# microsoft/VidTok

Hardware: NVIDIA H100
Metric: frames/sec encode+decode, kl_causal_488 17x256x256 (higher is better)
Workload: dtype bf16

## Files before the change

vidtok_b200/csrc/conv_tc.cu:

```cuda
#include <cuda.h>

#include <cstdio>
#include <cstdlib>
#include <cstring>
#include <mutex>
#include <string>
#include <type_traits>

#include "common.cuh"
#include "kernels.h"
#include "tc_host.h"
#include "tc_ptx.cuh"

namespace vt {

namespace {

thread_local std::string g_tc_err;

struct TcParams {
  int B, To, Ho, Wo, Co, Ti;
  int BW, BH, BT;
  int tilesW, tilesH, tilesT;
  int num_n_tiles, BN;
  long long num_tiles;
  int kt, kh, kw, Ci, num_kc;
  int st, pt, ph, pw, to_off;
  int sp;
  int t_mode, cacheT;
  int stages;
  const float* bias;
  int res_mode;
  const bf16* res;
  long long rsB, rsT, rsH, rsW;
  int resT, res_t_mode, res_pool_off;
  const bf16* res_cache;
  float ra, rb;
  void* out;
  long long osB, osT, osH, osW, osC;
  int out_f32;
  int Co_real;
  int w_batched;
  int ln_mode, ln_silu;
  const float* ln_gamma;
  const float* ln_beta;
  void* out2;
  int res_mma;
  int halo, hP, a_stages;
  uint32_t halo_bytes;
  int split, a_lo, b_lo, o_lo;
  float acc_scale;
  int kparts;
  int reg_mode, reg_zc, reg_sample;
  const float* reg_noise;
  float* reg_z;
  int* reg_idx;
  double* reg_kl;
  FsqConst reg_fsq;
  uint32_t misc_off;
};

struct TcMaps {
  CUtensorMap a[4];
  CUtensorMap c;
  CUtensorMap b;
  CUtensorMap r;
  CUtensorMap e;
};

constexpr int kConsumerWarps = 8;
constexpr int kProducerWarp = kConsumerWarps;
constexpr int kThreads = (kConsumerWarps + 4) * 32;
constexpr int kABytes = 128 * 128;
constexpr uint32_t kBarTurn = 3, kBarBias = 5;

__host__ __device__ constexpr bool ping_pong(int BN, bool split) { return !split && (BN == 64 || BN == 128); }

using namespace tcx;

struct TileCoord {
  int b, t0, h0, w0, n0;
};
__device__ __forceinline__ TileCoord decode_tile(const TcParams& p, long long tile) {
  TileCoord c;
  const int nt = (int)(tile % p.num_n_tiles);
  long long m = tile / p.num_n_tiles;
  const int tw = (int)(m % p.tilesW); m /= p.tilesW;
  const int th = (int)(m % p.tilesH); m /= p.tilesH;
  const int tt = (int)(m % p.tilesT);
  c.b = (int)(m / p.tilesT);
  c.t0 = tt * p.BT; c.h0 = th * p.BH; c.w0 = tw * p.BW; c.n0 = nt * p.BN;
  return c;
}
__device__ __forceinline__ bool tap_time(const TcParams& p, const TileCoord& tc, int a, int& tv, bool& from_cache) {
  tv = (tc.t0 + p.to_off) * p.st + a - p.pt;
  from_cache = false;
  if (tv + p.BT <= 0) {
    if (p.t_mode == 0) return false;
    if (p.t_mode == 1) { tv = 0; return true; }
    from_cache = true;
    tv = p.cacheT + tv;
    return true;
  }
  return true;
}
__device__ __forceinline__ int tile_taps(const TcParams& p, const TileCoord& tc) {
  int n = 0;
  for (int a = 0; a < p.kt; ++a) {
    int tv;
    bool from_cache;
    if (tap_time(p, tc, a, tv, from_cache)) ++n;
  }
  return n;
}

__device__ __forceinline__ float quad_sum(float v) {
  v += __shfl_xor_sync(0xffffffffu, v, 1);
  v += __shfl_xor_sync(0xffffffffu, v, 2);
  return v;
}

template <int BN, bool kSplit>
__global__ void __launch_bounds__(kThreads, 1)
conv_tc_kernel(const __grid_constant__ TcMaps maps, const TcParams p) {
  extern __shared__ uint8_t smem_raw[];
  const uint32_t smem_base = (smem_u32(smem_raw) + 1023u) & ~1023u;
  uint8_t* smem_gen = smem_raw + (smem_base - smem_u32(smem_raw));
  const int warp = threadIdx.x >> 5, lane = threadIdx.x & 31;
  const uint32_t a_bytes = kABytes;
  constexpr uint32_t b_bytes = (uint32_t)BN * 128u;
  constexpr uint32_t kPl = kSplit ? 2u : 1u;
  const uint32_t stage_bytes = kPl * (p.halo ? b_bytes : a_bytes + b_bytes);
  const uint32_t win_bytes = kPl * p.halo_bytes;
  const uint32_t ring_base = smem_base + (p.halo ? (uint32_t)p.a_stages * win_bytes : 0u);
  const uint32_t bar_base = ring_base + p.stages * stage_bytes;
  auto full_bar = [&](int s) { return bar_base + 8u * s; };
  auto empty_bar = [&](int s) { return bar_base + 8u * (p.stages + s); };
  auto fullA_bar = [&](int s) { return bar_base + 8u * (2 * p.stages + s); };
  auto emptyA_bar = [&](int s) { return bar_base + 8u * (2 * p.stages + p.a_stages + s); };
  constexpr bool kPingPong = ping_pong(BN, kSplit);
  float* sbias = reinterpret_cast<float*>(smem_gen + p.misc_off);
  float* rowbuf = sbias + 2 * 768;

  if (threadIdx.x == 0) {
    constexpr uint32_t readers = kPingPong ? kConsumerWarps / 2 : kConsumerWarps;
    for (int s = 0; s < p.stages; ++s) {
      mbar_init(full_bar(s), 1);
      mbar_init(empty_bar(s), readers);
    }
    for (int s = 0; s < p.a_stages; ++s) {
      mbar_init(fullA_bar(s), 1);
      mbar_init(emptyA_bar(s), readers);
    }
    asm volatile("fence.mbarrier_init.release.cluster;" ::: "memory");
  }
  __syncthreads();

  const int nsp = p.kh * p.kw;
  const int num_kc = p.num_kc, nstages = p.stages;
  const bool halo = p.halo != 0;
  const int res_steps = p.res_mma ? BN / 64 : 0;

  if (warp >= kProducerWarp) {
    asm volatile("setmaxnreg.dec.sync.aligned.u32 40;" ::: "memory");
    if (warp != kProducerWarp) return;
    const bool el = elect_one();
    if (el) {
      prefetch_tmap(&maps.a[0]);
      prefetch_tmap(&maps.b);
      if (p.sp == 2) { prefetch_tmap(&maps.a[1]); prefetch_tmap(&maps.a[2]); prefetch_tmap(&maps.a[3]); }
      if (p.t_mode == 2) prefetch_tmap(&maps.c);
      if (p.res_mma) { prefetch_tmap(&maps.r); prefetch_tmap(&maps.e); }
    }
    int stage = 0, sA = 0;
    uint32_t phase = 0, phA = 0;
    auto acquire = [&](uint32_t bytes) {
      mbar_wait(empty_bar(stage), phase ^ 1u);
      if (el) mbar_expect_tx(full_bar(stage), bytes);
    };
    auto advance = [&]() { if (++stage == nstages) { stage = 0; phase ^= 1u; } };
    auto load_b_planes = [&](uint32_t dst, const CUtensorMap* m, int kcol, int n, int wb_) {
      tma_load_3d(dst, m, full_bar(stage), kcol, n, wb_);
      if constexpr (kSplit) tma_load_3d(dst + b_bytes, m, full_bar(stage), p.b_lo + kcol, n, wb_);
    };
    auto load_window = [&](const CUtensorMap* m, int c0, int lo_off, int cw, int ch, int ct, int cb) {
      mbar_wait(emptyA_bar(sA), phA ^ 1u);
      if (el) {
        mbar_expect_tx(fullA_bar(sA), win_bytes);
        tma_load_5d(smem_base + (uint32_t)sA * win_bytes, m, fullA_bar(sA), c0, cw, ch, ct, cb);
        if constexpr (kSplit) tma_load_5d(smem_base + (uint32_t)sA * win_bytes + p.halo_bytes, m, fullA_bar(sA), lo_off + c0, cw, ch, ct, cb);
      }
      if (++sA == p.a_stages) { sA = 0; phA ^= 1u; }
    };
    for (long long tile = blockIdx.x; tile < p.num_tiles; tile += gridDim.x) {
      const TileCoord tc = decode_tile(p, tile);
      const int wb = p.w_batched ? tc.b : 0;
      for (int a = 0; a < p.kt; ++a) {
        int tv;
        bool from_cache;
        if (!tap_time(p, tc, a, tv, from_cache)) continue;
        if (halo) {
          const CUtensorMap* mapA = from_cache ? &maps.c : &maps.a[0];
          for (int kc = 0; kc < num_kc; ++kc) {
            load_window(mapA, kc * 64, p.a_lo, tc.w0 - p.pw, tc.h0 - p.ph, tv, tc.b);
            int kcol = a * nsp * p.Ci + kc * 64;
            for (int sp = 0; sp < nsp; ++sp, kcol += p.Ci) {
              acquire(stage_bytes);
              if (el) load_b_planes(ring_base + stage * stage_bytes, &maps.b, kcol, tc.n0, wb);
              advance();
            }
          }
        } else {
          int kcol = a * nsp * p.Ci;
          for (int bb = 0; bb < p.kh; ++bb) {
            for (int c = 0; c < p.kw; ++c, kcol += p.Ci) {
              const int dh = bb - p.ph, dw2 = c - p.pw;
              int ch, cw;
              const CUtensorMap* mapA;
              if (p.sp == 2) {
                mapA = &maps.a[(dh & 1) * 2 + (dw2 & 1)];
                ch = tc.h0 + (dh >> 1);
                cw = tc.w0 + (dw2 >> 1);
              } else {
                mapA = &maps.a[0];
                ch = tc.h0 + dh;
                cw = tc.w0 + dw2;
              }
              if (from_cache) mapA = &maps.c;
              for (int kc = 0; kc < num_kc; ++kc) {
                acquire(stage_bytes);
                if (el) {
                  const uint32_t sa = smem_base + stage * stage_bytes;
                  tma_load_5d(sa, mapA, full_bar(stage), kc * 64, cw, ch, tv, tc.b);
                  if constexpr (kSplit) tma_load_5d(sa + a_bytes, mapA, full_bar(stage), p.a_lo + kc * 64, cw, ch, tv, tc.b);
                  load_b_planes(sa + kPl * a_bytes, &maps.b, kcol + kc * 64, tc.n0, wb);
                }
                advance();
              }
            }
          }
        }
      }
      for (int g = 0; g < res_steps; ++g) {
        if (halo) {
          load_window(&maps.r, tc.n0 + g * 64, p.o_lo, tc.w0 - p.pw, tc.h0 - p.ph, tc.t0, tc.b);
          acquire(b_bytes);
          if (el) tma_load_3d(ring_base + stage * stage_bytes, &maps.e, full_bar(stage), g * 64, 0, 0);
        } else {
          acquire(kPl * a_bytes + b_bytes);
          if (el) {
            const uint32_t sa = smem_base + stage * stage_bytes;
            tma_load_5d(sa, &maps.r, full_bar(stage), tc.n0 + g * 64, tc.w0, tc.h0, tc.t0, tc.b);
            if constexpr (kSplit) tma_load_5d(sa + a_bytes, &maps.r, full_bar(stage), p.o_lo + tc.n0 + g * 64, tc.w0, tc.h0, tc.t0, tc.b);
            tma_load_3d(sa + kPl * a_bytes, &maps.e, full_bar(stage), g * 64, 0, 0);
          }
        }
        advance();
      }
    }
    return;
  }

  asm volatile("setmaxnreg.inc.sync.aligned.u32 232;" ::: "memory");
  constexpr int R = BN / 2;
  constexpr int kHalves = kPingPong ? 2 : 1;
  constexpr bool kSum = kSplit && BN <= 128;
  const int g = warp >> 2, wq = warp & 3;
  const bool leader = lane == 0;
  const uint32_t hi_b = desc_hi(1024u);
  const uint32_t hi_a = halo ? desc_hi((uint32_t)p.hP * 128u) : hi_b;
  const uint32_t a_half = halo ? 8u * (uint32_t)p.hP * 128u : 64u * 128u;
  const uint32_t a_row_off = kPingPong ? 0u : (uint32_t)g * a_half;
  const uint32_t a_pl = halo ? p.halo_bytes : a_bytes;
  const uint32_t b_addr0 = halo ? ring_base : smem_base + kPl * a_bytes;
  float acc[kHalves][R];
  float sum[kSum ? R : 1];
  int stage = 0, sA = 0, sR = 0;
  uint32_t phase = 0, phA = 0;
  int pend_stage = -1;
  bool pend_win = false;
  auto release = [&]() {
    if (leader) {
      if (pend_stage >= 0) mbar_arrive(empty_bar(pend_stage));
      if (pend_win) mbar_arrive(emptyA_bar(sR));
    }
    if (pend_win && ++sR == p.a_stages) sR = 0;
    pend_stage = -1;
    pend_win = false;
  };
  auto kstep = [&](bool a_from_stage, uint32_t a_addr, uint32_t scale, bool res, bool last_of_window) {
    mbar_wait(full_bar(stage), phase);
    if (a_from_stage) a_addr = smem_base + stage * stage_bytes + a_row_off;
    const uint32_t b_addr = b_addr0 + stage * stage_bytes;
    const uint32_t al = desc_lo(a_addr), bl = desc_lo(b_addr);
    wgmma_fence();
#pragma unroll
    for (uint32_t j = 0; j < 4u; ++j) {
      const uint64_t ah = desc(al + 2u * j, hi_a), bh = desc(bl + 2u * j, hi_b);
      wgmma_k16<BN, kSplit>(acc[0], ah, bh, j == 0 ? scale : 1u);
      if constexpr (kPingPong) wgmma_k16<BN, kSplit>(acc[1], desc(al + (a_half >> 4) + 2u * j, hi_a), bh, j == 0 ? scale : 1u);
      if constexpr (kSplit) {
        wgmma_k16<BN, kSplit>(acc[0], desc(al + (a_pl >> 4) + 2u * j, hi_a), bh, 1u);
        if (!res) wgmma_k16<BN, kSplit>(acc[0], ah, desc(bl + (b_bytes >> 4) + 2u * j, hi_b), 1u);
      }
    }
    wgmma_commit();
    wgmma_wait<1>();
    release();
    pend_stage = stage;
    pend_win = last_of_window;
    if (++stage == nstages) { stage = 0; phase ^= 1u; }
  };

  const int rbase = (kPingPong ? 0 : 64 * g) + 16 * wq + (lane >> 2);
  const int cq = 2 * (lane & 3);
  const bool res_direct = (p.res_mode == 1 && !p.res_mma);
  const bool store_a = (p.ln_mode != 1);
  const float inv_n = 1.0f / (float)BN;
  int last_n0 = -1;
  uint32_t cbuf = 1;

  int owner = 0;
  for (long long tile = blockIdx.x; tile < p.num_tiles; tile += gridDim.x, owner ^= 1) {
    const TileCoord tc = decode_tile(p, tile);
    if constexpr (kPingPong) {
      if (owner != g) {
        const int taps = tile_taps(p, tc);
        stage += taps * nsp * num_kc + res_steps;
        if ((stage / nstages) & 1) phase ^= 1u;
        stage %= nstages;
        if (halo) {
          const int nw = taps * num_kc + res_steps;
          sA += nw;
          if ((sA / p.a_stages) & 1) phA ^= 1u;
          sA %= p.a_stages;
          sR = (sR + nw) % p.a_stages;
        }
        continue;
      }
      if (tile != blockIdx.x) named_bar_sync(kBarTurn + g, kConsumerWarps * 32);
    }
    uint32_t G = 0xFFFFFFFFu;
    if constexpr (kSum) {
      if (p.kparts > 1) {
        const uint32_t nk = (uint32_t)(tile_taps(p, tc) * nsp * num_kc + res_steps);
        G = (nk + (uint32_t)p.kparts - 1u) / (uint32_t)p.kparts;
      }
#pragma unroll
      for (int i = 0; i < R; ++i) sum[i] = 0.f;
    }
    uint32_t ks = 0, accum = 0;
    auto step = [&](bool a_from_stage, uint32_t a_addr, bool res, bool last_of_window) {
      if constexpr (kSum) {
        if (ks > 0 && ks % G == 0) {
          wgmma_wait<0>();
          acc_fence(acc[0]);
          release();
#pragma unroll
          for (int i = 0; i < R; ++i) sum[i] += acc[0][i];
          accum = 0;
        }
      }
      kstep(a_from_stage, a_addr, accum, res, last_of_window);
      accum = 1;
      ++ks;
    };
    for (int a = 0; a < p.kt; ++a) {
      int tv;
      bool from_cache;
      if (!tap_time(p, tc, a, tv, from_cache)) continue;
      if (halo) {
        for (int kc = 0; kc < num_kc; ++kc) {
          mbar_wait(fullA_bar(sA), phA);
          const uint32_t win = smem_base + (uint32_t)sA * win_bytes + a_row_off;
          for (int bb = 0; bb < p.kh; ++bb)
            for (int c = 0; c < p.kw; ++c)
              step(false, win + (uint32_t)(bb * p.hP + c) * 128u, false, bb == p.kh - 1 && c == p.kw - 1);
          if (++sA == p.a_stages) { sA = 0; phA ^= 1u; }
        }
      } else {
        for (int s = nsp * num_kc; s > 0; --s) step(true, 0u, false, false);
      }
    }
    for (int gr = 0; gr < res_steps; ++gr) {
      if (halo) {
        mbar_wait(fullA_bar(sA), phA);
        step(false, smem_base + (uint32_t)sA * win_bytes + a_row_off + (uint32_t)(p.ph * p.hP + p.pw) * 128u, true, true);
        if (++sA == p.a_stages) { sA = 0; phA ^= 1u; }
      } else {
        step(true, 0u, true, false);
      }
    }
    if constexpr (kPingPong) {
      if (tile + gridDim.x < p.num_tiles) named_bar_arrive(kBarTurn + (g ^ 1), kConsumerWarps * 32);
    }
    wgmma_wait<0>();
#pragma unroll
    for (int hf = 0; hf < kHalves; ++hf) acc_fence(acc[hf]);
    release();
    if constexpr (kSum) {
#pragma unroll
      for (int i = 0; i < R; ++i) acc[0][i] += sum[i];
    }

    if (tc.n0 != last_n0) {
      last_n0 = tc.n0;
      cbuf ^= 1u;
      constexpr int nthr = kPingPong ? 128 : kConsumerWarps * 32;
      float* b_ = sbias + ((kPingPong ? 2 * g : 0) + cbuf) * 768;
      for (int i = threadIdx.x % nthr; i < BN; i += nthr) {
        b_[i] = (p.bias && tc.n0 + i < p.Co_real) ? p.bias[tc.n0 + i] : 0.f;
        if (p.ln_mode) { const float sc = (p.ln_silu && !kSplit) ? 0.5f : 1.0f; b_[256 + i] = sc * p.ln_gamma[tc.n0 + i]; b_[512 + i] = sc * p.ln_beta[tc.n0 + i]; }
      }
      named_bar_sync(kPingPong ? kBarBias + g : 1u, nthr);
    }
    const float* bias_s = sbias + ((kPingPong ? 2 * g : 0) + cbuf) * 768;
    const float* gamma_s = bias_s + 256;
    const float* beta_s = bias_s + 512;

#pragma unroll
    for (int hf = 0; hf < kHalves; ++hf) {
      float (&acc_h)[R] = acc[hf];
      int row0 = rbase + 64 * hf;
      asm volatile("" : "+r"(row0));
      bool valid[2];
      long long ooff[2];
      auto row_geom = [&](int row, int& t, int& h, int& w) {
        const int dw = halo ? (row & 7) : row % p.BW;
        const int dh = halo ? (row >> 3) : (row / p.BW) % p.BH;
        const int dt = halo ? 0 : row / (p.BW * p.BH);
        t = tc.t0 + dt; h = tc.h0 + dh; w = tc.w0 + dw;
        return (t < p.To) && (h < p.Ho) && (w < p.Wo);
      };
#pragma unroll
      for (int r = 0; r < 2; ++r) {
        int t, h, w;
        valid[r] = row_geom(row0 + 8 * r, t, h, w);
        ooff[r] = (long long)tc.b * p.osB + (long long)t * p.osT + (long long)h * p.osH + (long long)w * p.osW;
      }
      auto res_pair = [&](const bf16* rp, int c, float& x0, float& x1) {
        const uint32_t hw = *reinterpret_cast<const uint32_t*>(rp + c);
        if constexpr (kSplit) {
          const uint32_t lw = *reinterpret_cast<const uint32_t*>(rp + p.o_lo + c);
          x0 = f16_lo(hw) + f16_lo(lw);
          x1 = f16_hi(hw) + f16_hi(lw);
        } else {
          x0 = bf16_lo(hw);
// ... 268 lines not shown
  }
  if (reg && reg->mode) {
    const int need = reg->mode == 1 ? 2 * reg->zc : reg->zc;
    const bool zc_ok = reg->mode == 1 ? (reg->zc == 4 || reg->zc == 8 || reg->zc == 16) : reg->zc <= VT_MAX_FSQ;
    if (tout == DT_F32 && Co_pad == 32 && need <= p.Co && zc_ok && p.osW == 1) t.reg = *reg;
    else g_tc_err = "regularizer epilogue needs an fp32 [B,C,T,H,W] head with Cout <= 32 holding all latent channels";
  }
  auto plan = [&](bool allow_halo, int bn_cap) -> int {
    t.halo = 0; t.hP = 0; t.a_stages = 0; t.halo_bytes = 0;
    t.BN = choose_bn(Co_pad);
    if (bn_cap && t.BN > bn_cap) t.BN = bn_cap;
    if (!choose_tile(p, 128, t.BW, t.BH, t.BT)) { g_tc_err = "no tile shape"; return -1; }
    const bool geom = p.sh == 1 && p.sw == 1 && p.kh * p.kw > 1 && p.kh <= 3 && p.kw <= 3 && p.Ho == p.Hi && p.Wo == p.Wi &&
                      w_batches <= 1 && p.Wo % 8 == 0 && p.Ho % 16 == 0;
    if (allow_halo && geom) {
      t.halo = 1;
      t.BW = 8; t.BH = 16; t.BT = 1;
      t.hP = 16;
      t.halo_bytes = (uint32_t)((16 + p.kh - 1) * t.hP * 128);
      t.a_stages = 2;
    }
    const size_t stage_bytes = (size_t)cw * ((t.halo ? 0 : (size_t)kABytes) + (size_t)t.BN * 128);
    const size_t budget = 225 * 1024;
    const size_t a_ring = (size_t)t.a_stages * t.halo_bytes * cw;
    const size_t misc = (ping_pong(t.BN, split) ? 4 : 2) * 768 * 4 + (t.reg.mode ? 128 * 33 * 4 : 0);
    const size_t fixed = 1024  + misc + 16;
    if (budget < fixed + a_ring + 2 * (stage_bytes + 16)) return 1;
    int stages = (int)((budget - fixed - a_ring) / (stage_bytes + 16));
    if (stages > 8) stages = 8;
    static const int cap = [] { const char* e = getenv("VT_TC_STAGES"); return e ? atoi(e) : 0; }();
    if (cap >= 2 && stages > cap) stages = cap;
    t.stages = stages;
    const size_t bars = 8 * (2 * (size_t)stages + 2 * (size_t)t.a_stages);
    t.misc_off = (uint32_t)((a_ring + stages * stage_bytes + bars + 15) & ~(size_t)15);
    t.smem = 1024 + t.misc_off + misc;
    t.kparts = (split && t.BN <= 128 && nk >= 16) ? (nk >= 64 ? 8 : 4) : 1;
    return 0;
  };
  const bool need_row = t.ln.mode != 0;
  const int bn_pref = (split && !need_row && w_batches <= 1) ? (nk >= 128 ? 64 : (nk >= 16 ? 128 : 0)) : 0;
  int rc = plan(true, bn_pref);
  if (rc == 1) rc = plan(false, bn_pref);
  if (rc == 1 && !need_row) rc = plan(false, 128);
  if (rc == 1) return no("not enough shared memory for 2 stages");
  if (rc != 0) return false;
  bool ident_ok = true;
  if (split) {
    const float ws = p.acc_scale != 0.f ? 1.0f / p.acc_scale : 1.0f;
    t.ident_s = ilogbf(ws);
    ident_ok = t.ident_s >= 0 && t.ident_s <= 15 && ldexpf(1.0f, t.ident_s) == ws;
  }
  t.res_mma = (ident_ok && p.res_mode == 1 && p.ra == 1.0f && p.rb == 1.0f && t.BN % 64 == 0 && p.Co % 64 == 0 && p.rsW % 8 == 0 &&
               p.rsH % 8 == 0 && p.rsT % 8 == 0 && p.rsB % 8 == 0 && (((uintptr_t)p.res) & 15) == 0) ? 1 : 0;
  *out = t;
  return true;
}

cudaError_t launch_conv_tc(const TcPlan& pl, const bf16* x, const bf16* w_nk, void* out, cudaStream_t s, long long w_batch_stride) {
  if (!tmap_encoder()) { g_tc_err = "cuTensorMapEncodeTiled unavailable"; return cudaErrorNotSupported; }
  const ConvP& p = pl.p;
  const TcRegFusion& reg = pl.reg;
  const bool split = p.split != 0;
  const int cw = split ? 2 : 1;
  if (reg.mode ? (!reg.z || (reg.mode == 1 && (!reg.kl_acc || (reg.sample && !reg.noise)))) : !out) { g_tc_err = "null output"; return cudaErrorInvalidValue; }
  if (p.t_mode == 2 && (!p.cache || p.cacheT <= 0)) { g_tc_err = "cache mode without cache"; return cudaErrorInvalidValue; }
  int dev = 0;
  const cudaError_t dev_err = current_device(dev);
  if (dev_err != cudaSuccess) { g_tc_err = "no current device, or its index is out of range"; return dev_err; }
  const int Co_pad = (p.Co + 31) / 32 * 32, Kpad = p.kt * p.kh * p.kw * p.Ci;
  TcParams t;
  memset(&t, 0, sizeof(t));
  t.BW = pl.BW; t.BH = pl.BH; t.BT = pl.BT; t.BN = pl.BN;
  t.halo = pl.halo; t.hP = pl.hP; t.a_stages = pl.a_stages; t.halo_bytes = pl.halo_bytes;
  t.stages = pl.stages; t.misc_off = pl.misc_off; t.kparts = pl.kparts; t.res_mma = pl.res_mma;
  t.tilesW = (p.Wo + t.BW - 1) / t.BW; t.tilesH = (p.Ho + t.BH - 1) / t.BH; t.tilesT = (p.To + t.BT - 1) / t.BT;
  t.num_n_tiles = Co_pad / t.BN;
  t.num_tiles = (long long)p.B * t.tilesT * t.tilesH * t.tilesW * t.num_n_tiles;
  t.split = split ? 1 : 0; t.a_lo = p.Ci; t.b_lo = Kpad; t.o_lo = p.Co;
  t.acc_scale = (split && p.acc_scale != 0.f) ? p.acc_scale : 1.0f;
  t.B = p.B; t.To = p.To; t.Ho = p.Ho; t.Wo = p.Wo; t.Co = p.Co; t.Ti = p.Ti;
  t.kt = p.kt; t.kh = p.kh; t.kw = p.kw; t.Ci = p.Ci; t.num_kc = p.Ci / 64;
  t.st = p.st; t.pt = p.pt; t.ph = p.ph; t.pw = p.pw; t.to_off = p.to_off; t.sp = p.sh;
  t.t_mode = p.t_mode; t.cacheT = p.cacheT;
  t.bias = p.bias; t.res_mode = p.res_mode; t.res = (const bf16*)p.res;
  t.rsB = p.rsB; t.rsT = p.rsT; t.rsH = p.rsH; t.rsW = p.rsW; t.resT = p.resT; t.res_t_mode = p.res_t_mode; t.res_pool_off = p.res_pool_off;
  t.res_cache = (const bf16*)p.res_cache; t.ra = p.ra; t.rb = p.rb;
  t.out = out; t.osB = p.osB; t.osT = p.osT; t.osH = p.osH; t.osW = p.osW; t.osC = p.osC;
  t.out_f32 = (pl.tout == DT_F32) ? 1 : 0;
  t.Co_real = p.Co;
  t.ln_mode = pl.ln.mode; t.ln_silu = pl.ln.silu ? 1 : 0; t.ln_gamma = pl.ln.gamma; t.ln_beta = pl.ln.beta; t.out2 = pl.ln.out2;
  if (reg.mode) {
    t.reg_mode = reg.mode; t.reg_zc = reg.zc; t.reg_sample = reg.sample; t.reg_noise = reg.noise; t.reg_z = reg.z;
    t.reg_idx = reg.indices; t.reg_kl = reg.kl_acc;
    if (reg.mode == 2) t.reg_fsq = make_fsq_const(reg.zc, reg.fsq_levels);
  }
  t.w_batched = pl.w_batches > 1 ? 1 : 0;

  TcMaps maps;
  auto encode_act = [&](CUtensorMap* m, const bf16* base, int Wn, int Hn, long long sw_, long long sh_, int Tn, long long st_, long long bs) -> bool {
    cuuint64_t dims[5] = {(cuuint64_t)(cw * p.Ci), (cuuint64_t)Wn, (cuuint64_t)Hn, (cuuint64_t)Tn, (cuuint64_t)p.B};
    cuuint64_t strides[4] = {(cuuint64_t)sw_ * 2, (cuuint64_t)sh_ * 2, (cuuint64_t)st_ * 2, (cuuint64_t)bs * 2};
    cuuint32_t box[5] = {64, (cuuint32_t)t.BW, (cuuint32_t)t.BH, (cuuint32_t)t.BT, 1};
    if (t.halo) { box[1] = (cuuint32_t)t.hP; box[2] = (cuuint32_t)(16 + p.kh - 1); }
    return encode_tmap_16b(m, 5, base, dims, strides, box, "activation", g_tc_err);
  };
  if (p.sh == 1) {
    if (!encode_act(&maps.a[0], x, p.Wi, p.Hi, p.isW, p.isH, p.Ti, p.isT, p.isB)) return cudaErrorInvalidValue;
    maps.a[1] = maps.a[2] = maps.a[3] = maps.a[0];
  } else {
    for (int hp = 0; hp < 2; ++hp)
      for (int wp = 0; wp < 2; ++wp)
        if (!encode_act(&maps.a[hp * 2 + wp], x + (long long)hp * p.isH + (long long)wp * p.isW, (p.Wi - wp + 1) / 2,
                        (p.Hi - hp + 1) / 2, 2 * p.isW, 2 * p.isH, p.Ti, p.isT, p.isB))
          return cudaErrorInvalidValue;
  }
  if (p.t_mode == 2) {
    if (!encode_act(&maps.c, (const bf16*)p.cache, p.Wi, p.Hi, p.isW, p.isH, p.cacheT, p.isT, (long long)p.cacheT * p.Hi * p.Wi * p.Ci * cw)) return cudaErrorInvalidValue;
  } else {
    maps.c = maps.a[0];
  }
  {
    const int nb = pl.w_batches > 1 ? pl.w_batches : 1;
    cuuint64_t dims[3] = {(cuuint64_t)(cw * Kpad), (cuuint64_t)Co_pad, (cuuint64_t)nb};
    cuuint64_t strides[2] = {(cuuint64_t)(cw * Kpad) * 2, (cuuint64_t)(nb > 1 ? w_batch_stride : (long long)cw * Kpad * Co_pad) * 2};
    cuuint32_t box[3] = {64, (cuuint32_t)t.BN, 1};
    if (!encode_tmap_16b(&maps.b, 3, w_nk, dims, strides, box, "weights", g_tc_err)) return cudaErrorInvalidValue;
  }
  auto encode_out = [&](CUtensorMap* m, const void* base, int Tn, long long sW, long long sH, long long sT, long long sB, int bw, int bh, int bt) -> bool {
    cuuint64_t dims[5] = {(cuuint64_t)(cw * p.Co), (cuuint64_t)p.Wo, (cuuint64_t)p.Ho, (cuuint64_t)Tn, (cuuint64_t)p.B};
    cuuint64_t strides[4] = {(cuuint64_t)sW * 2, (cuuint64_t)sH * 2, (cuuint64_t)sT * 2, (cuuint64_t)sB * 2};
    cuuint32_t box[5] = {64, (cuuint32_t)bw, (cuuint32_t)bh, (cuuint32_t)bt, 1};
    return encode_tmap_16b(m, 5, base, dims, strides, box, "output/residual", g_tc_err);
  };
  maps.r = maps.a[0]; maps.e = maps.b;
  if (t.res_mma) {
    static bf16* ident_dev[2][kMaxDevices] = {{nullptr}};
    static std::mutex ident_mu;
    const int ik = split ? 1 : 0;
    {
      std::lock_guard<std::mutex> lock(ident_mu);
      if (!ident_dev[ik][dev]) {
        const int nmat = split ? 16 : 1;
        bf16* e = nullptr;
        cudaError_t err = cudaMalloc(&e, (size_t)nmat * 256 * 256 * sizeof(bf16));
        if (err != cudaSuccess) { g_tc_err = "cudaMalloc(identity)"; return err; }
        for (int i = 0; i < nmat; ++i) fill_identity_kernel<<<256, 256, 0, s>>>(e + (size_t)i * 256 * 256, ik, ldexpf(1.0f, i));
        if ((err = cudaStreamSynchronize(s)) != cudaSuccess) { cudaFree(e); g_tc_err = "identity fill"; return err; }
        ident_dev[ik][dev] = e;
      }
    }
    const bf16* ident = ident_dev[ik][dev] + (size_t)pl.ident_s * 256 * 256;
    if (!encode_out(&maps.r, p.res, p.resT, p.rsW, p.rsH, p.rsT, p.rsB, t.halo ? t.hP : t.BW, t.halo ? 16 + p.kh - 1 : t.BH, t.BT)) return cudaErrorInvalidValue;
    cuuint64_t dims[3] = {256, 256, 1};
    cuuint64_t strides[2] = {512, 256 * 512};
    cuuint32_t box[3] = {64, (cuuint32_t)t.BN, 1};
    if (!encode_tmap_16b(&maps.e, 3, ident, dims, strides, box, "identity", g_tc_err)) return cudaErrorInvalidValue;
  }
  {
    static SmemLimitOnce smem_limit;
    cudaError_t e = smem_limit.ensure(dev, 227 * 1024, conv_tc_kernel<32, false>, conv_tc_kernel<64, false>, conv_tc_kernel<128, false>,
                                      conv_tc_kernel<256, false>, conv_tc_kernel<32, true>, conv_tc_kernel<64, true>,
                                      conv_tc_kernel<128, true>, conv_tc_kernel<256, true>);
    if (e != cudaSuccess) { g_tc_err = "cudaFuncSetAttribute(smem)"; return e; }
  }
  const int num_sms = device_sms(dev);
  const unsigned grid = (unsigned)(t.num_tiles < num_sms ? t.num_tiles : num_sms);
  const double Mrows = (double)p.B * p.To * p.Ho * p.Wo;
  char det[160] = "";
  if (prof_enabled()) snprintf(det, sizeof(det), "k%d%d%d s%d%d %d->%d @%dx%dx%d tile%dx%dx%d bn%d%s ln%d r%d%s p%d t%d st%d", p.kt, p.kh, p.kw, p.st, p.sh, p.Ci, p.Co, p.To, p.Ho, p.Wo, t.BT, t.BH, t.BW, t.BN, t.halo ? " halo" : "", t.ln_mode, p.res_mode, t.res_mma ? "m" : "", split ? t.kparts : 1, p.t_mode, t.stages);
  ProfScope _ps(split ? "conv_tc3" : "conv_tc", 2.0 * Mrows * p.kt * p.kh * p.kw * p.Ci * p.Co,
                2.0 * cw * ((double)p.B * p.Ti * p.Hi * p.Wi * p.Ci) + Mrows * p.Co * (pl.tout == DT_F32 ? 4.0 : 2.0 * cw), s, det);
  auto launch = [&](auto kern) { kern<<<grid, kThreads, pl.smem, s>>>(maps, t); };
  switch (t.BN * 2 + (split ? 1 : 0)) {
    case 64: launch(conv_tc_kernel<32, false>); break;
    case 65: launch(conv_tc_kernel<32, true>); break;
    case 128: launch(conv_tc_kernel<64, false>); break;
    case 129: launch(conv_tc_kernel<64, true>); break;
    case 256: launch(conv_tc_kernel<128, false>); break;
    case 257: launch(conv_tc_kernel<128, true>); break;
    case 512: launch(conv_tc_kernel<256, false>); break;
    default: launch(conv_tc_kernel<256, true>); break;
  }
  count_launch();
  return cudaGetLastError();
}

}
```

vidtok_b200/csrc/kernels.h:

```cpp
#pragma once
#include <cuda_runtime.h>
#include <stdint.h>

#include "common.cuh"

namespace vt {

enum DType { DT_F32 = 0, DT_BF16 = 1, DT_SPLIT = 2 };
inline size_t dtype_size(DType t) { return t == DT_BF16 ? 2 : 4; }

void prof_start();
void prof_set_detail(bool on);
int prof_stop(char* buf, int cap);

cudaError_t launch_conv_simt(const ConvP& p, DType tin, DType tout, DType tres, const void* x, const float* w_kn,
                             void* out, cudaStream_t s);
cudaError_t launch_gemm_simt(DType ta, DType tb, DType tc, const void* A, const void* B, void* C, int M, int N, int K,
                             long long lda, long long sbn, long long sbk, long long ldc, int batch, long long bsA,
                             long long bsB, long long bsC, float scale, cudaStream_t s);

cudaError_t launch_layernorm(DType t, const void* x, const float* gamma, const float* beta, void* y, long long rows,
                             int C, bool silu, bool exact, cudaStream_t s);
cudaError_t launch_groupnorm(DType t, const void* x, const float* gamma, const float* beta, void* y, long long frames,
                             long long pos_per_frame, int C, bool per_position, bool silu, bool exact, float* stats,
// ... 26 lines not shown
                                  float wscale = 0.f);
cudaError_t launch_absmax(const float* w, long long n, float* out, cudaStream_t s);
inline float split_weight_scale(float maxabs, float headroom = 1.0f) {
  if (!(maxabs > 0.f)) return 1.0f;
  float sc = 1.0f;
  while (sc * maxabs * headroom < 2048.0f && sc < 1.0e30f) sc *= 2.0f;
  while (sc * maxabs * headroom >= 4096.0f && sc > 1.0e-30f) sc *= 0.5f;
  return sc;
}
constexpr float kModelWeightHeadroom = 4.0f;
cudaError_t launch_pack_w_collapsed(const float* w, bf16* out, int Co, int Co_pad, int Ci, int kt, int kh, int kw,
                                    const int* mt, const int* mh, const int* mw, int kt2, int kh2, int kw2, cudaStream_t s,
                                    float wscale = 0.f);
cudaError_t launch_time_interp2x(DType t, const void* x, void* y, int B, int T, long long hw, int C, cudaStream_t s);
cudaError_t launch_upsample_nearest(DType t, const void* x, void* y, int B, int T, int H, int W, int C, int ut, int uh,
                                    int uw, cudaStream_t s);
cudaError_t launch_cache_update(DType t, const void* x, const void* old_cache, void* new_cache, int B, int Tc, int P,
                                int off, bool first, long long frame_elems, long long x_bs, cudaStream_t s);
cudaError_t launch_ncdhw_to_cl(DType t, const float* x, void* y, int B, int C, int T, int H, int W, int t_rep,
                               cudaStream_t s);
cudaError_t launch_copy_frames(DType t, const void* src, void* dst, int B, long long src_bs, long long dst_bs,
                               long long n_per_batch, cudaStream_t s);

cudaError_t launch_u8_frames_to_clip(const uint8_t* src, float* dst, int T, int Hs, int Ws, int C, int h0, int w0, int H, int W,
                                    cudaStream_t s);
cudaError_t launch_clip_to_u8_frames(const float* src, uint8_t* dst, int C, int T, int H, int W, cudaStream_t s);
bool u8_frames_resize_fits(int Hs, int Ws, int C, int Hr, int Wr, int h0, int w0, int H, int W);
cudaError_t launch_u8_frames_resize_to_clip(const uint8_t* src, float* dst, int N, int Hs, int Ws, int C, int Hr, int Wr, int h0,
                                            int w0, int H, int W, int Tc, cudaStream_t s);
cudaError_t launch_split_to_f32(const bf16* x, float* y, long long rows, int C, cudaStream_t s);
cudaError_t launch_f32_to_split(const float* x, bf16* y, long long rows, int C, cudaStream_t s);

struct TcLnFusion {
  int mode = 0;
  bool silu = true;
  const float* gamma = nullptr;
  const float* beta = nullptr;
  void* out2 = nullptr;
};
struct TcRegFusion {
  int mode = 0;
  int zc = 0;
  int sample = 1;
  const float* noise = nullptr;
  float* z = nullptr;
  int* indices = nullptr;
  double* kl_acc = nullptr;
  int fsq_levels[VT_MAX_FSQ] = {0};
};
struct TcPlan {
  ConvP p;
  DType tout;
  int w_batches, BN, BW, BH, BT, halo, hP, a_stages, stages, kparts, res_mma, ident_s;
  uint32_t halo_bytes, misc_off;
  size_t smem;
  TcLnFusion ln;
  TcRegFusion reg;
};
bool conv_tc_plan(const ConvP& p, DType tout, const TcLnFusion* ln, const TcRegFusion* reg, int w_batches, TcPlan* out);
cudaError_t launch_conv_tc(const TcPlan& pl, const bf16* x, const bf16* w_nk, void* out, cudaStream_t s, long long w_batch_stride = 0);
cudaError_t launch_kl_clear(double* scratch, cudaStream_t s);
cudaError_t launch_kl_finish(const double* scratch, int B, float* kl_loss, cudaStream_t s);
cudaError_t launch_tap_planes_gather(const bf16* P, const float* bias, float* out, int B, int Ti, int H, int W, int NP, int Co,
                                     int to_off, cudaStream_t s, int pt = 2);
cudaError_t launch_pack_w_tap_planes(const float* w, bf16* out, int Co, int Ci, int NP, cudaStream_t s);
cudaError_t launch_transpose_bf16(const bf16* x, bf16* y, int batch, int rows, int cols, cudaStream_t s, bool split = false);
const char* conv_tc_last_error();

bool tblock_tc_supported(int B, int T, int H, int W, int C);
struct TbCache {
  const bf16* n1_in = nullptr;
  const bf16* h_in = nullptr;
  bf16* n1_out = nullptr;
  bf16* h_out = nullptr;
};
cudaError_t launch_tblock_tc(const bf16* n1, const bf16* x, const bf16* w1, const float* bias1, const float* gamma2,
                             const float* beta2, const bf16* w2, const float* bias2, bf16* out, bf16* out2,
                             const float* gamma_out, const float* beta_out, bool out_silu, int B, int T, int H, int W,
                             cudaStream_t s, const TbCache* cache = nullptr);
const char* tblock_tc_last_error();

bool attn_tc_supported(long long frames, long long tokens, int C, bool split);
size_t attn_tc_workspace(long long frames, long long tokens, int C, bool split);
cudaError_t launch_attn_tc(const bf16* q, const bf16* k, const bf16* v, bf16* o, int frames, int H, int W, int C, bool split,
                           void* ws, cudaStream_t s);
const char* attn_tc_last_error();

bool conv_stem_supported(const ConvP& p);
cudaError_t launch_conv_stem(const ConvP& p, const float* x, const bf16* wpk, bf16* out, cudaStream_t s);
cudaError_t launch_stem_cache_update(const float* x, float* cache, int B, int Ci, int T, int t_rep, int H, int W, cudaStream_t s);

}
```

vidtok_b200/csrc/tc_host.h:

```cpp
#pragma once
#include <cuda.h>
#include <cuda_runtime.h>

#include <atomic>
#include <string>

namespace vt {

constexpr int kMaxDevices = 64;

typedef CUresult (*EncodeTiledFn)(CUtensorMap*, CUtensorMapDataType, cuuint32_t, void*, const cuuint64_t*,
                                  const cuuint64_t*, const cuuint32_t*, const cuuint32_t*, CUtensorMapInterleave,
                                  CUtensorMapSwizzle, CUtensorMapL2promotion, CUtensorMapFloatOOBfill);

inline EncodeTiledFn tmap_encoder() {
  static const EncodeTiledFn fn = [] {
    void* f = nullptr;
    cudaDriverEntryPointQueryResult q;
    const bool ok = cudaGetDriverEntryPoint("cuTensorMapEncodeTiled", &f, cudaEnableDefault, &q) == cudaSuccess &&
                    q == cudaDriverEntryPointSuccess;
    return ok ? (EncodeTiledFn)f : nullptr;
  }();
  return fn;
}

inline bool encode_tmap_16b(CUtensorMap* map, int rank, const void* base, const cuuint64_t* dims, const cuuint64_t* strides,
                            const cuuint32_t* box, const char* what, std::string& err) {
  const EncodeTiledFn enc = tmap_encoder();
  if (!enc) { err = "cuTensorMapEncodeTiled unavailable"; return false; }
  const cuuint32_t elem_strides[5] = {1, 1, 1, 1, 1};
  const CUresult r = enc(map, CU_TENSOR_MAP_DATA_TYPE_BFLOAT16, (cuuint32_t)rank, const_cast<void*>(base), dims, strides, box,
                         elem_strides, CU_TENSOR_MAP_INTERLEAVE_NONE, CU_TENSOR_MAP_SWIZZLE_128B,
                         CU_TENSOR_MAP_L2_PROMOTION_L2_256B, CU_TENSOR_MAP_FLOAT_OOB_FILL_NONE);
  if (r != CUDA_SUCCESS) { err = std::string("cuTensorMapEncodeTiled(") + what + ") failed: " + std::to_string((int)r); return false; }
  return true;
}

inline cudaError_t current_device(int& dev) {
  const cudaError_t e = cudaGetDevice(&dev);
  if (e != cudaSuccess) return e;
  return dev >= 0 && dev < kMaxDevices ? cudaSuccess : cudaErrorInvalidDevice;
}

inline int device_sms(int dev) {
  static std::atomic<int> sms[kMaxDevices];
  int n = sms[dev].load(std::memory_order_relaxed);
  if (n == 0) {
    cudaDeviceGetAttribute(&n, cudaDevAttrMultiProcessorCount, dev);
    if (n <= 0) n = 132;
    sms[dev].store(n, std::memory_order_relaxed);
  }
  return n;
}

class SmemLimitOnce {
 public:
  template <class... Kernels>
  cudaError_t ensure(int dev, int bytes, Kernels... kernels) {
    if (done_[dev].load(std::memory_order_acquire)) return cudaSuccess;
    cudaError_t e = cudaSuccess;
    for (const void* k : {(const void*)kernels...}) {
      const cudaError_t x = cudaFuncSetAttribute(k, cudaFuncAttributeMaxDynamicSharedMemorySize, bytes);
      if (x != cudaSuccess) e = x;
    }
    if (e == cudaSuccess) done_[dev].store(true, std::memory_order_release);
    return e;
  }

 private:
  std::atomic<bool> done_[kMaxDevices] = {};
};

}
```

vidtok_b200/csrc/tc_ptx.cuh:

```cuda
#pragma once
#include <cuda.h>
#include <cuda_bf16.h>
#include <cuda_fp16.h>
#include <stdint.h>

namespace vt {
namespace tcx {
__device__ __forceinline__ uint32_t smem_u32(const void* p) { return (uint32_t)__cvta_generic_to_shared(p); }

__device__ __forceinline__ void mbar_init(uint32_t bar, uint32_t count) {
  asm volatile("mbarrier.init.shared::cta.b64 [%0], %1;" ::"r"(bar), "r"(count) : "memory");
}
__device__ __forceinline__ void mbar_expect_tx(uint32_t bar, uint32_t bytes) {
  asm volatile("mbarrier.arrive.expect_tx.shared::cta.b64 _, [%0], %1;" ::"r"(bar), "r"(bytes) : "memory");
}
__device__ __forceinline__ void mbar_arrive(uint32_t bar) {
  asm volatile("mbarrier.arrive.shared::cta.b64 _, [%0];" ::"r"(bar) : "memory");
}
__device__ __forceinline__ bool mbar_try_wait(uint32_t bar, uint32_t parity) {
  uint32_t ok;
  asm volatile(
      "{\n\t"
      ".reg .pred p;\n\t"
      "mbarrier.try_wait.parity.shared::cta.b64 p, [%1], %2;\n\t"
      "selp.u32 %0, 1, 0, p;\n\t"
      "}"
      : "=r"(ok)
      : "r"(bar), "r"(parity)
      : "memory");
  return ok != 0;
}
__device__ __forceinline__ void mbar_wait(uint32_t bar, uint32_t parity) {
  if (mbar_try_wait(bar, parity)) return;
  const long long t0 = clock64();
  while (!mbar_try_wait(bar, parity)) {
    if (clock64() - t0 > 8000000000LL) __trap();
  }
}
__device__ __forceinline__ void tma_load_5d(uint32_t dst, const CUtensorMap* map, uint32_t bar, int c0, int c1, int c2,
                                            int c3, int c4) {
  asm volatile(
      "cp.async.bulk.tensor.5d.shared::cluster.global.mbarrier::complete_tx::bytes [%0], [%1, {%3, %4, %5, %6, %7}], [%2];"
      ::"r"(dst), "l"(map), "r"(bar), "r"(c0), "r"(c1), "r"(c2), "r"(c3), "r"(c4)
      : "memory");
}
__device__ __forceinline__ void tma_load_3d(uint32_t dst, const CUtensorMap* map, uint32_t bar, int c0, int c1, int c2) {
  asm volatile(
      "cp.async.bulk.tensor.3d.shared::cluster.global.mbarrier::complete_tx::bytes [%0], [%1, {%3, %4, %5}], [%2];"
      ::"r"(dst), "l"(map), "r"(bar), "r"(c0), "r"(c1), "r"(c2)
      : "memory");
}
__device__ __forceinline__ void tma_store_5d(const CUtensorMap* map, uint32_t src, int c0, int c1, int c2, int c3, int c4) {
  asm volatile("cp.async.bulk.tensor.5d.global.shared::cta.bulk_group [%0, {%2, %3, %4, %5, %6}], [%1];"
               ::"l"(map), "r"(src), "r"(c0), "r"(c1), "r"(c2), "r"(c3), "r"(c4)
               : "memory");
}
__device__ __forceinline__ void bulk_commit() { asm volatile("cp.async.bulk.commit_group;" ::: "memory"); }
template <int kPending>
__device__ __forceinline__ void bulk_wait_read() { asm volatile("cp.async.bulk.wait_group.read %0;" ::"n"(kPending) : "memory"); }
template <int kPending>
__device__ __forceinline__ void bulk_wait() { asm volatile("cp.async.bulk.wait_group %0;" ::"n"(kPending) : "memory"); }
__device__ __forceinline__ void fence_async_smem() { asm volatile("fence.proxy.async.shared::cta;" ::: "memory"); }
__device__ __forceinline__ void named_bar_sync(uint32_t id, uint32_t threads) {
  asm volatile("bar.sync %0, %1;" ::"r"(id), "r"(threads) : "memory");
}
__device__ __forceinline__ void named_bar_arrive(uint32_t id, uint32_t threads) {
  asm volatile("bar.arrive %0, %1;" ::"r"(id), "r"(threads) : "memory");
}
__device__ __forceinline__ void prefetch_tmap(const CUtensorMap* map) {
  asm volatile("prefetch.tensormap [%0];" ::"l"(map) : "memory");
}
__device__ __forceinline__ bool elect_one() {
  uint32_t pred;
  asm volatile(
      "{\n\t"
      ".reg .pred P1;\n\t"
      "elect.sync _|P1, 0xffffffff;\n\t"
      "selp.u32 %0, 1, 0, P1;\n\t"
      "}"
      : "=r"(pred));
  return pred != 0;
}

__device__ __forceinline__ void wgmma_fence() { asm volatile("wgmma.fence.sync.aligned;" ::: "memory"); }
__device__ __forceinline__ void wgmma_commit() { asm volatile("wgmma.commit_group.sync.aligned;" ::: "memory"); }
template <int kPending>
__device__ __forceinline__ void wgmma_wait() { asm volatile("wgmma.wait_group.sync.aligned %0;" ::"n"(kPending) : "memory"); }
template <int R>
__device__ __forceinline__ void acc_fence(float (&d)[R]) {
#pragma unroll
  for (int i = 0; i < R; ++i) asm volatile("" : "+f"(d[i])::"memory");
}

__device__ __forceinline__ uint32_t desc_lo(uint32_t saddr) { return ((saddr & 0x3FFFFu) >> 4) | (1u << 16); }
__device__ __forceinline__ uint32_t desc_hi(uint32_t sbo) { return (sbo >> 4) | (1u << 30); }
__device__ __forceinline__ uint64_t desc(uint32_t lo, uint32_t hi) { return ((uint64_t)hi << 32) | lo; }

__device__ __forceinline__ void wgmma_32_bf16(float (&d)[16], uint64_t da, uint64_t db, uint32_t scale_d) {
  asm volatile(
      "{\n\t.reg .pred p;\n\t"
      "setp.ne.b32 p, %18, 0;\n\t"
      "wgmma.mma_async.sync.aligned.m64n32k16.f32.bf16.bf16 "
      "{"
// ... 203 lines not shown
```

Measured before the change: 458.3.

## Multicast conv weight tiles across 2-CTA clusters via TMA

Launches the tensor-core conv kernel as 2-CTA clusters that pair adjacent W tiles. Each CTA loads half of the weight (B) tile and multicasts it to both CTAs, which halves weight traffic from L2. Empty barriers now count consumers from both CTAs through remote cluster arrives, and the producer drains the pipeline before exiting. The trade-off is extra cluster synchronisation coupling the two CTAs and possible scheduling constraints from cluster occupancy. The grid is sized with cudaOccupancyMaxActiveClusters.

```diff
diff --git a/vidtok_b200/csrc/conv_tc.cu b/vidtok_b200/csrc/conv_tc.cu
--- a/vidtok_b200/csrc/conv_tc.cu
+++ b/vidtok_b200/csrc/conv_tc.cu
@@ -21,9 +21,10 @@
 struct TcParams {
   int B, To, Ho, Wo, Co, Ti;
   int BW, BH, BT;
-  int tilesW, tilesH, tilesT;
+  int groupsW, tilesH, tilesT;
   int num_n_tiles, BN;
-  long long num_tiles;
+  int cl, group_step;
+  long long num_groups;
   int kt, kh, kw, Ci, num_kc;
   int st, pt, ph, pw, to_off;
   int sp;
@@ -72,6 +73,7 @@
 constexpr int kProducerWarp = kConsumerWarps;
 constexpr int kThreads = (kConsumerWarps + 4) * 32;
 constexpr int kABytes = 128 * 128;
+constexpr int kCluster = 2;
 constexpr uint32_t kBarTurn = 3, kBarBias = 5;
 
 __host__ __device__ constexpr bool ping_pong(int BN, bool split) { return !split && (BN == 64 || BN == 128); }
@@ -81,11 +83,11 @@
 struct TileCoord {
   int b, t0, h0, w0, n0;
 };
-__device__ __forceinline__ TileCoord decode_tile(const TcParams& p, long long tile) {
+__device__ __forceinline__ TileCoord decode_tile(const TcParams& p, long long q) {
   TileCoord c;
-  const int nt = (int)(tile % p.num_n_tiles);
-  long long m = tile / p.num_n_tiles;
-  const int tw = (int)(m % p.tilesW); m /= p.tilesW;
+  const int nt = (int)(q % p.num_n_tiles);
+  long long m = q / p.num_n_tiles;
+  const int tw = (int)(m % p.groupsW) * p.cl + (int)(blockIdx.x % (unsigned)p.cl); m /= p.groupsW;
   const int th = (int)(m % p.tilesH); m /= p.tilesH;
   const int tt = (int)(m % p.tilesT);
   c.b = (int)(m / p.tilesT);
@@ -146,7 +148,7 @@
     constexpr uint32_t readers = kPingPong ? kConsumerWarps / 2 : kConsumerWarps;
     for (int s = 0; s < p.stages; ++s) {
       mbar_init(full_bar(s), 1);
-      mbar_init(empty_bar(s), readers);
+      mbar_init(empty_bar(s), readers * (uint32_t)p.cl);
     }
     for (int s = 0; s < p.a_stages; ++s) {
       mbar_init(fullA_bar(s), 1);
@@ -154,7 +156,10 @@
     }
     asm volatile("fence.mbarrier_init.release.cluster;" ::: "memory");
   }
-  __syncthreads();
+  const int cl = p.cl;
+  if (cl > 1) cluster_sync();
+  else __syncthreads();
+  const long long q0 = cl > 1 ? blockIdx.x / kCluster : blockIdx.x;
 
   const int nsp = p.kh * p.kw;
   const int num_kc = p.num_kc, nstages = p.stages;
@@ -180,8 +185,17 @@
     };
     auto advance = [&]() { if (++stage == nstages) { stage = 0; phase ^= 1u; } };
     auto load_b_planes = [&](uint32_t dst, const CUtensorMap* m, int kcol, int n, int wb_) {
-      tma_load_3d(dst, m, full_bar(stage), kcol, n, wb_);
-      if constexpr (kSplit) tma_load_3d(dst + b_bytes, m, full_bar(stage), p.b_lo + kcol, n, wb_);
+      if (cl > 1) {
+        constexpr int rows = BN / kCluster;
+        constexpr uint16_t all = (1u << kCluster) - 1u;
+        const int r0 = (int)(blockIdx.x % kCluster) * rows;
+        const uint32_t d = dst + (uint32_t)r0 * 128u;
+        tma_load_3d_multicast(d, m, full_bar(stage), all, kcol, n + r0, wb_);
+        if constexpr (kSplit) tma_load_3d_multicast(d + b_bytes, m, full_bar(stage), all, p.b_lo + kcol, n + r0, wb_);
+      } else {
+        tma_load_3d(dst, m, full_bar(stage), kcol, n, wb_);
+        if constexpr (kSplit) tma_load_3d(dst + b_bytes, m, full_bar(stage), p.b_lo + kcol, n, wb_);
+      }
     };
     auto load_window = [&](const CUtensorMap* m, int c0, int lo_off, int cw, int ch, int ct, int cb) {
       mbar_wait(emptyA_bar(sA), phA ^ 1u);
@@ -192,8 +206,8 @@
       }
       if (++sA == p.a_stages) { sA = 0; phA ^= 1u; }
     };
-    for (long long tile = blockIdx.x; tile < p.num_tiles; tile += gridDim.x) {
-      const TileCoord tc = decode_tile(p, tile);
+    for (long long q = q0; q < p.num_groups; q += p.group_step) {
+      const TileCoord tc = decode_tile(p, q);
       const int wb = p.w_batched ? tc.b : 0;
       for (int a = 0; a < p.kt; ++a) {
         int tv;
@@ -258,6 +272,12 @@
         advance();
       }
     }
+    if (cl > 1) {
+      for (int i = 0; i < nstages; ++i) {
+        mbar_wait(empty_bar(stage), phase ^ 1u);
+        advance();
+      }
+    }
     return;
   }
 
@@ -281,7 +301,11 @@
   bool pend_win = false;
   auto release = [&]() {
     if (leader) {
-      if (pend_stage >= 0) mbar_arrive(empty_bar(pend_stage));
+      if (pend_stage >= 0) {
+#pragma unroll
+        for (int c = 0; c < kCluster; ++c)
+          if (c < p.cl) mbar_arrive_cluster(empty_bar(pend_stage), (uint32_t)c);
+      }
       if (pend_win) mbar_arrive(emptyA_bar(sR));
     }
     if (pend_win && ++sR == p.a_stages) sR = 0;
@@ -321,8 +345,8 @@
   uint32_t cbuf = 1;
 
   int owner = 0;
-  for (long long tile = blockIdx.x; tile < p.num_tiles; tile += gridDim.x, owner ^= 1) {
-    const TileCoord tc = decode_tile(p, tile);
+  for (long long q = q0; q < p.num_groups; q += p.group_step, owner ^= 1) {
+    const TileCoord tc = decode_tile(p, q);
     if constexpr (kPingPong) {
       if (owner != g) {
         const int taps = tile_taps(p, tc);
@@ -338,7 +362,7 @@
         }
         continue;
       }
-      if (tile != blockIdx.x) named_bar_sync(kBarTurn + g, kConsumerWarps * 32);
+      if (q >= p.group_step) named_bar_sync(kBarTurn + g, kConsumerWarps * 32);
     }
     uint32_t G = 0xFFFFFFFFu;
     if constexpr (kSum) {
@@ -392,7 +416,7 @@
       }
     }
     if constexpr (kPingPong) {
-      if (tile + gridDim.x < p.num_tiles) named_bar_arrive(kBarTurn + (g ^ 1), kConsumerWarps * 32);
+      if (q + p.group_step < p.num_groups) named_bar_arrive(kBarTurn + (g ^ 1), kConsumerWarps * 32);
     }
     wgmma_wait<0>();
 #pragma unroll
@@ -767,6 +791,9 @@
   }
   t.res_mma = (ident_ok && p.res_mode == 1 && p.ra == 1.0f && p.rb == 1.0f && t.BN % 64 == 0 && p.Co % 64 == 0 && p.rsW % 8 == 0 &&
                p.rsH % 8 == 0 && p.rsT % 8 == 0 && p.rsB % 8 == 0 && (((uintptr_t)p.res) & 15) == 0) ? 1 : 0;
+  static const int cl_cap = [] { const char* e = getenv("VT_TC_CLUSTER"); return e ? atoi(e) : 0; }();
+  const int tilesW = (p.Wo + t.BW - 1) / t.BW;
+  t.cluster = (tilesW % kCluster == 0 && w_batches <= 1 && !(cl_cap >= 1 && cl_cap < kCluster)) ? kCluster : 1;
   *out = t;
   return true;
 }
@@ -787,10 +814,10 @@
   memset(&t, 0, sizeof(t));
   t.BW = pl.BW; t.BH = pl.BH; t.BT = pl.BT; t.BN = pl.BN;
   t.halo = pl.halo; t.hP = pl.hP; t.a_stages = pl.a_stages; t.halo_bytes = pl.halo_bytes;
-  t.stages = pl.stages; t.misc_off = pl.misc_off; t.kparts = pl.kparts; t.res_mma = pl.res_mma;
-  t.tilesW = (p.Wo + t.BW - 1) / t.BW; t.tilesH = (p.Ho + t.BH - 1) / t.BH; t.tilesT = (p.To + t.BT - 1) / t.BT;
+  t.stages = pl.stages; t.misc_off = pl.misc_off; t.kparts = pl.kparts; t.res_mma = pl.res_mma; t.cl = pl.cluster;
+  t.groupsW = (p.Wo + t.BW - 1) / t.BW / t.cl; t.tilesH = (p.Ho + t.BH - 1) / t.BH; t.tilesT = (p.To + t.BT - 1) / t.BT;
   t.num_n_tiles = Co_pad / t.BN;
-  t.num_tiles = (long long)p.B * t.tilesT * t.tilesH * t.tilesW * t.num_n_tiles;
+  t.num_groups = (long long)p.B * t.tilesT * t.tilesH * t.groupsW * t.num_n_tiles;
   t.split = split ? 1 : 0; t.a_lo = p.Ci; t.b_lo = Kpad; t.o_lo = p.Co;
   t.acc_scale = (split && p.acc_scale != 0.f) ? p.acc_scale : 1.0f;
   t.B = p.B; t.To = p.To; t.Ho = p.Ho; t.Wo = p.Wo; t.Co = p.Co; t.Ti = p.Ti;
@@ -838,7 +865,7 @@
     const int nb = pl.w_batches > 1 ? pl.w_batches : 1;
     cuuint64_t dims[3] = {(cuuint64_t)(cw * Kpad), (cuuint64_t)Co_pad, (cuuint64_t)nb};
     cuuint64_t strides[2] = {(cuuint64_t)(cw * Kpad) * 2, (cuuint64_t)(nb > 1 ? w_batch_stride : (long long)cw * Kpad * Co_pad) * 2};
-    cuuint32_t box[3] = {64, (cuuint32_t)t.BN, 1};
+    cuuint32_t box[3] = {64, (cuuint32_t)(t.BN / t.cl), 1};
     if (!encode_tmap_16b(&maps.b, 3, w_nk, dims, strides, box, "weights", g_tc_err)) return cudaErrorInvalidValue;
   }
   auto encode_out = [&](CUtensorMap* m, const void* base, int Tn, long long sW, long long sH, long long sT, long long sB, int bw, int bh, int bt) -> bool {
@@ -878,24 +905,48 @@
                                       conv_tc_kernel<128, true>, conv_tc_kernel<256, true>);
     if (e != cudaSuccess) { g_tc_err = "cudaFuncSetAttribute(smem)"; return e; }
   }
-  const int num_sms = device_sms(dev);
-  const unsigned grid = (unsigned)(t.num_tiles < num_sms ? t.num_tiles : num_sms);
+  void (*kern)(TcMaps, TcParams);
+  switch (t.BN * 2 + (split ? 1 : 0)) {
+    case 64: kern = conv_tc_kernel<32, false>; break;
+    case 65: kern = conv_tc_kernel<32, true>; break;
+    case 128: kern = conv_tc_kernel<64, false>; break;
+    case 129: kern = conv_tc_kernel<64, true>; break;
+    case 256: kern = conv_tc_kernel<128, false>; break;
+    case 257: kern = conv_tc_kernel<128, true>; break;
+    case 512: kern = conv_tc_kernel<256, false>; break;
+    default: kern = conv_tc_kernel<256, true>; break;
+  }
+  unsigned grid;
+  if (t.cl == 1) {
+    const int num_sms = device_sms(dev);
+    grid = (unsigned)(t.num_groups < num_sms ? t.num_groups : num_sms);
+  } else {
+    static ActiveClustersOnce active;
+    int clusters = 0;
+    const cudaError_t e = active.get(dev, (const void*)kern, kThreads, 227 * 1024, t.cl, clusters);
+    if (e != cudaSuccess) { g_tc_err = "cudaOccupancyMaxActiveClusters"; return e; }
+    grid = (unsigned)(t.cl * (t.num_groups < clusters ? t.num_groups : clusters));
+  }
+  t.group_step = (int)grid / t.cl;
   const double Mrows = (double)p.B * p.To * p.Ho * p.Wo;
   char det[160] = "";
   if (prof_enabled()) snprintf(det, sizeof(det), "k%d%d%d s%d%d %d->%d @%dx%dx%d tile%dx%dx%d bn%d%s ln%d r%d%s p%d t%d st%d", p.kt, p.kh, p.kw, p.st, p.sh, p.Ci, p.Co, p.To, p.Ho, p.Wo, t.BT, t.BH, t.BW, t.BN, t.halo ? " halo" : "", t.ln_mode, p.res_mode, t.res_mma ? "m" : "", split ? t.kparts : 1, p.t_mode, t.stages);
   ProfScope _ps(split ? "conv_tc3" : "conv_tc", 2.0 * Mrows * p.kt * p.kh * p.kw * p.Ci * p.Co,
                 2.0 * cw * ((double)p.B * p.Ti * p.Hi * p.Wi * p.Ci) + Mrows * p.Co * (pl.tout == DT_F32 ? 4.0 : 2.0 * cw), s, det);
-  auto launch = [&](auto kern) { kern<<<grid, kThreads, pl.smem, s>>>(maps, t); };
-  switch (t.BN * 2 + (split ? 1 : 0)) {
-    case 64: launch(conv_tc_kernel<32, false>); break;
-    case 65: launch(conv_tc_kernel<32, true>); break;
-    case 128: launch(conv_tc_kernel<64, false>); break;
-    case 129: launch(conv_tc_kernel<64, true>); break;
-    case 256: launch(conv_tc_kernel<128, false>); break;
-    case 257: launch(conv_tc_kernel<128, true>); break;
-    case 512: launch(conv_tc_kernel<256, false>); break;
-    default: launch(conv_tc_kernel<256, true>); break;
-  }
+  cudaLaunchAttribute attr;
+  attr.id = cudaLaunchAttributeClusterDimension;
+  attr.val.clusterDim.x = (unsigned)t.cl;
+  attr.val.clusterDim.y = 1;
+  attr.val.clusterDim.z = 1;
+  cudaLaunchConfig_t cfg = {};
+  cfg.gridDim = dim3(grid);
+  cfg.blockDim = dim3(kThreads);
+  cfg.dynamicSmemBytes = pl.smem;
+  cfg.stream = s;
+  cfg.attrs = &attr;
+  cfg.numAttrs = t.cl > 1 ? 1 : 0;
+  const cudaError_t e = cudaLaunchKernelEx(&cfg, kern, maps, t);
+  if (e != cudaSuccess) { g_tc_err = "conv_tc launch"; return e; }
   count_launch();
   return cudaGetLastError();
 }
diff --git a/vidtok_b200/csrc/kernels.h b/vidtok_b200/csrc/kernels.h
--- a/vidtok_b200/csrc/kernels.h
+++ b/vidtok_b200/csrc/kernels.h
@@ -102,6 +102,7 @@
   ConvP p;
   DType tout;
   int w_batches, BN, BW, BH, BT, halo, hP, a_stages, stages, kparts, res_mma, ident_s;
+  int cluster;
   uint32_t halo_bytes, misc_off;
   size_t smem;
   TcLnFusion ln;
diff --git a/vidtok_b200/csrc/tc_host.h b/vidtok_b200/csrc/tc_host.h
--- a/vidtok_b200/csrc/tc_host.h
+++ b/vidtok_b200/csrc/tc_host.h
@@ -53,6 +53,33 @@
   return n;
 }
 
+class ActiveClustersOnce {
+ public:
+  cudaError_t get(int dev, const void* kernel, int threads, int smem, int size, int& clusters) {
+    clusters = n_[dev].load(std::memory_order_relaxed);
+    if (clusters > 0) return cudaSuccess;
+    cudaLaunchAttribute attr;
+    attr.id = cudaLaunchAttributeClusterDimension;
+    attr.val.clusterDim.x = (unsigned)size;
+    attr.val.clusterDim.y = 1;
+    attr.val.clusterDim.z = 1;
+    cudaLaunchConfig_t cfg = {};
+    cfg.gridDim = dim3((unsigned)size);
+    cfg.blockDim = dim3((unsigned)threads);
+    cfg.dynamicSmemBytes = (size_t)smem;
+    cfg.attrs = &attr;
+    cfg.numAttrs = 1;
+    const cudaError_t e = cudaOccupancyMaxActiveClusters(&clusters, kernel, &cfg);
+    if (e != cudaSuccess) return e;
+    if (clusters <= 0) return cudaErrorInvalidConfiguration;
+    n_[dev].store(clusters, std::memory_order_relaxed);
+    return cudaSuccess;
+  }
+
+ private:
+  std::atomic<int> n_[kMaxDevices] = {};
+};
+
 class SmemLimitOnce {
  public:
   template <class... Kernels>
diff --git a/vidtok_b200/csrc/tc_ptx.cuh b/vidtok_b200/csrc/tc_ptx.cuh
--- a/vidtok_b200/csrc/tc_ptx.cuh
+++ b/vidtok_b200/csrc/tc_ptx.cuh
@@ -49,6 +49,26 @@
       "cp.async.bulk.tensor.3d.shared::cluster.global.mbarrier::complete_tx::bytes [%0], [%1, {%3, %4, %5}], [%2];"
       ::"r"(dst), "l"(map), "r"(bar), "r"(c0), "r"(c1), "r"(c2)
       : "memory");
+}
+__device__ __forceinline__ void tma_load_3d_multicast(uint32_t dst, const CUtensorMap* map, uint32_t bar, uint16_t cta_mask,
+                                                      int c0, int c1, int c2) {
+  asm volatile(
+      "cp.async.bulk.tensor.3d.shared::cluster.global.mbarrier::complete_tx::bytes.multicast::cluster [%0], [%1, {%4, %5, %6}], [%2], %3;"
+      ::"r"(dst), "l"(map), "r"(bar), "h"(cta_mask), "r"(c0), "r"(c1), "r"(c2)
+      : "memory");
+}
+__device__ __forceinline__ void mbar_arrive_cluster(uint32_t bar, uint32_t cta) {
+  asm volatile(
+      "{\n\t"
+      ".reg .b32 ra;\n\t"
+      "mapa.shared::cluster.u32 ra, %0, %1;\n\t"
+      "mbarrier.arrive.shared::cluster.b64 _, [ra];\n\t"
+      "}"
+      ::"r"(bar), "r"(cta)
+      : "memory");
+}
+__device__ __forceinline__ void cluster_sync() {
+  asm volatile("barrier.cluster.arrive.release;\n\tbarrier.cluster.wait.acquire;" ::: "memory");
 }
 __device__ __forceinline__ void tma_store_5d(const CUtensorMap* map, uint32_t src, int c0, int c1, int c2, int c3, int c4) {
   asm volatile("cp.async.bulk.tensor.5d.global.shared::cta.bulk_group [%0, {%2, %3, %4, %5, %6}], [%1];"
```

New measurement: 464.7, median of 6. 1.4% higher.
